# Sara-H-dev/Semantic_Segmentation_Of_StyleGAN2_Artifacts

Measured on AMD Instinct MI355X. Metric: training images/sec at 1024^2 bs=8 per GPU (MS-UNet Swin-T, fwd+DynamicLoss+bwd+AdamW), higher is better.
Workload: dtype bf16; 1 GPU; 1xMI355X 1024x1024 bs=8 Swin-T MS-UNet train step; model=MS-UNet swin_t, global_batch=8, world_size=1, img_size=1024, parallelism=dp1, grad_allreduce=f32, dead_branches=executed (no grad), step_execution=eager, params=42881040

## Files before the change

### include/msunet_hip.h

```cpp
#ifndef MSUNET_HIP_H
#define MSUNET_HIP_H

#ifdef __cplusplus
extern "C" {
#endif

int msu_layernorm_fwd(int dtype, int mode, const void* x, const void* b, const float* bscale,
                      long rows_per_sample, void* s_out, const float* gamma, const float* beta,
                      void* y, float* mean, float* rstd, long rows, int C, int H, int W, int Cin,
                      float eps, void* stream);
int msu_layernorm_bwd(int dtype, int mode, const void* dy, const void* x, const void* dres,
                      const float* gamma, const float* mean, const float* rstd, void* dx,
                      void* db, const float* bscale, long rows_per_sample, float* part,
                      int nparts, float* dgamma, float* dbeta, long rows, int C, int H, int W,
                      int Cin, int accumulate, void* stream);
int msu_layernorm_bwd3(int dtype, int mode, const void* dy, const void* x, const void* dres,
                       const void* dres2, const void* dres3, const float* gamma, const float* mean,
                       const float* rstd, void* dx, void* db, const float* bscale, long rows_per_sample,
                       float* part, int nparts, float* dgamma, float* dbeta, long rows, int C, int H, int W,
                       int Cin, int accumulate, void* stream);
int msu_ln_part_blocks(long rows, int C);
int msu_colsum_batch(int nseg, const float* const* part, const long* stride, const int* nparts, const int* n,
                     float* const* out, int accumulate, void* stream);
int msu_tail_reduce_mode(int mode);
// ... 77 lines not shown
int msu_tok_gemm_supported(long M, int N, int K);
int msu_tok_gemm_supported_epi(long M, int N, int K, int epi);
int msu_tok_gemm(int dtype, const void* A, const void* A2, int K1, const void* W, const float* bias, void* Y,
                 void* Y2, const void* H, long M, int N, int K, int epi, void* stream);
int msu_tok_gemm_plan(long M, int N, int K, long* out6);
int msu_tok_gemm_plan_epi(long M, int N, int K, int epi, int concat, long* out6);
int msu_nt_gemm_supported(long M, int N, int K);
int msu_nt_gemm_plan(long M, int N);
int msu_nt_gemm_plan2(long M, int N, int K, int epi, int wkn, long* out8);
int msu_nt_gemm_mode(int mode);
int msu_nt_gemm(int dtype, const void* A, const void* W, const float* bias, void* Y, void* Y2, const void* H,
                long M, int N, int K, int epi, void* stream);
int msu_nt_gemm_cat(int dtype, const void* A, const void* A2, int K1, const void* W, const float* bias, void* Y,
                    long M, int N, int K, void* stream);
int msu_nt_gemm_kn(int dtype, const void* A, const void* Wk, const float* bias, void* Y, void* Y2, const void* H,
                   long M, int N, int K, int epi, void* stream);

int msu_mlp_fused_supported(int C, int Hd);
int msu_add_ln_mlp_fwd(int dtype, const void* a, const void* br, const float* bscale, long rows_per_sample,
                       const float* gamma, const float* beta, float eps, const void* w1, const float* b1,
                       const void* w2, const float* b2, void* s_out, void* y, long M, int C, int Hd, void* stream);
int msu_mlp_fused_fwd(int dtype, const void* x, const void* w1, const float* b1, const void* w2, const float* b2,
                      void* y, void* h, long M, int C, int Hd, void* stream);
int msu_gelu_fwd(int dtype, const void* x, void* y, long n, void* stream);
int msu_gelu_bwd(int dtype, const void* x, const void* dy, void* dx, long n, void* stream);
int msu_transpose16_multi(const void* src, void* dst, const long long* table, int nent, int ntiles,
                          void* stream);
int msu_residual(int dtype, const void* a, const void* b, const float* scale, void* out, long n, long per_sample,
                 void* stream);
int msu_patchify(int dtype, const float* img, void* out, int B, int Cin, int H, int W, int p,
                 void* stream);

int msu_dynloss_nblk(long N);
int msu_dynloss_fwd(int dtype, const void* logits, const float* target, int B, long N,
                    float alpha, float beta, float mix, float* part, int nblk, float* loss,
                    float* coef, void* stream);
int msu_dynloss_bwd(int dtype, const void* logits, const float* target, const float* coef,
                    const float* loss, const float* gout, int B, long N, float alpha, float beta,
                    float mix, float* dlogits, void* stream);
int msu_dynloss_fwd2(int dtype, const void* logits, const float* target, int B, long N,
                     float alpha, float beta, float mix, float* part, int nblk, float* loss, float* flag,
                     float* coef, void* stream);
int msu_dynloss_bwd2(int dtype, const void* logits, const float* target, const float* coef,
                     const float* flag, const float* gout, int B, long N, float alpha, float beta,
                     float mix, float* dlogits, void* stream);
int msu_dynloss_fwd3(int dtype, const void* logits, const float* target, int B, long N,
// ... 53 lines not shown
```

### semantic_segmentation_of_stylegan2_artifacts_amd/_lib.py

```python
import ctypes
import os

from . import switches

_HERE = os.path.dirname(os.path.abspath(__file__))
LIB_PATH = switches.get("MSU_LIB_OVERRIDE") or os.path.join(_HERE, "libmsunet_hip.so")

P = ctypes.c_void_p
I = ctypes.c_int
L = ctypes.c_long
F = ctypes.c_float
D = ctypes.c_double
U64 = ctypes.c_ulonglong

SIGNATURES = {
    "msu_ln_part_blocks": (I, [L, I]),
    "msu_layernorm_fwd": (I, [I, I, P, P, P, L, P, P, P, P, P, P, L, I, I, I, I, F, P]),
    "msu_layernorm_bwd": (I, [I, I, P, P, P, P, P, P, P, P, P, L, P, I, P, P, L, I, I, I, I, I, P]),
    "msu_layernorm_bwd3": (I, [I, I, P, P, P, P, P, P, P, P, P, P, P, L, P, I, P, P, L, I, I, I, I, I, P]),
    "msu_reduce_rows": (I, [P, I, I, L, P, I, P]),
    "msu_tail_reduce_mode": (I, [I]),
    "msu_conv_mode": (I, [I]),
    "msu_conv3x3_route": (I, [I, I, I]),
    "msu_head_fwd": (I, [I, P, P, P, P, P, P, P, L, I, F, P]),
    "msu_head_bwd": (I, [I, P, P, P, P, P, P, P, P, P, I, P, P, P, L, I, P]),
    "msu_head_bwd2": (I, [I, P, P, P, P, P, P, P, P, P, I, P, P, P, L, I, I, P]),
    "msu_win_count": (L, [I, I, I]),
    "msu_win_attn_fwd_workspace": (L, [I, I, I]),
    "msu_win_attn_keep_words": (L, [I, I, I, I, I]),
    "msu_win_attn_fwd": (I, [I, P, P, P, P, P, I, I, I, I, I, I, F, U64, P, P, P]),
    "msu_win_attn_bwd_workspace": (L, [I, I, I, I, I, I]),
    "msu_win_attn_bwd": (I, [I, P, P, P, P, P, P, P, P, I, I, I, I, I, I, F, U64, P, P, P]),
    "msu_win_attn_bwd2": (I, [I, P, P, P, P, P, P, P, P, I, I, I, I, I, I, F, U64, P, P, P, P]),
    "msu_win_attn_bwd_tail": (I, [I, P, P, P, I, I, I, I, I, P]),
    "msu_win_attn_bwd_tail2": (I, [I, P, P, P, I, I, I, I, I, I, P]),
    "msu_win_attn_qkv_supported": (I, [I, I]),
    "msu_win_attn_qkv_fwd": (I, [I, P, P, P, P, P, P, P, P, I, I, I, I, I, I, F, U64, P, P]),
    "msu_win_attn_qkv_fwd2": (I, [I, P, P, P, P, P, P, P, P, P, P, P, I, I, I, I, I, I, F, U64, P, P]),
    "msu_mlp_fused_supported": (I, [I, I]),
    "msu_mlp_fused_fwd": (I, [I, P, P, P, P, P, P, P, L, I, I, P]),
    "msu_add_ln_mlp_fwd": (I, [I, P, P, P, L, P, P, F, P, P, P, P, P, P, L, I, I, P]),
    "msu_gelu_fwd": (I, [I, P, P, L, P]),
    "msu_gelu_bwd": (I, [I, P, P, P, L, P]),
    "msu_residual": (I, [I, P, P, P, P, L, L, P]),
    "msu_patchify": (I, [I, P, P, I, I, I, I, I, P]),
    "msu_dynloss_nblk": (I, [L]),
    "msu_dynloss_fwd": (I, [I, P, P, I, L, F, F, F, P, I, P, P, P]),
    "msu_dynloss_bwd": (I, [I, P, P, P, P, P, I, L, F, F, F, P, P]),
    "msu_dynloss_fwd2": (I, [I, P, P, I, L, F, F, F, P, I, P, P, P, P]),
    "msu_dynloss_fwd3": (I, [I, P, P, I, L, F, F, F, P, I, P, P, P, P, P]),
    "msu_dynloss_bwd2": (I, [I, P, P, P, P, P, I, L, F, F, F, P, P]),
    "msu_adamw": (I, [P, P, P, P, L, F, F, F, F, F, I, P, P, P]),
    "msu_nonfinite": (I, [P, L, P, P]),
    "msu_nonfinite2": (I, [P, L, P, L, P, P]),
    "msu_grad_sumsq_nblk": (I, [L]),
    "msu_grad_sumsq2": (I, [P, L, P, L, P, I, P, P]),
    "msu_grad_clip_scale": (I, [P, I, P, D, P, P, P]),
    "msu_adamw_dev": (I, [P, P, P, P, L, P, D, D, D, D, P, P, P]),
    "msu_adamw_dev2": (I, [P, P, P, P, L, P, D, D, D, D, P, P, P, I, I, P]),
    "msu_adamw_dev3": (I, [P, P, P, P, P, L, P, D, D, D, D, D, P, P, P, I, I, P]),
    "msu_swap_cast": (I, [P, P, P, I, L, P]),
    "msu_step_advance": (I, [P, P, P]),
    "msu_loss_scale_step": (I, [P, P, P, P, P, P, D, D, I, P]),
# ... 76 lines not shown
```

### semantic_segmentation_of_stylegan2_artifacts_amd/csrc/common.h

```cpp
#pragma once
#include <hip/hip_runtime.h>
#include <hip/hip_bf16.h>
#include <stdint.h>

#include <mutex>

#define MSU_DEV __device__ __forceinline__

typedef __bf16 bf16x8 __attribute__((ext_vector_type(8)));
typedef float f32x4 __attribute__((ext_vector_type(4)));
typedef float f32x16 __attribute__((ext_vector_type(16)));
typedef uint32_t u32x4 __attribute__((ext_vector_type(4)));
typedef uint32_t u32x2 __attribute__((ext_vector_type(2)));
typedef float f32x2 __attribute__((ext_vector_type(2)));
typedef uint16_t bf16_t;
typedef _Float16 f16_t;
typedef _Float16 f16x8 __attribute__((ext_vector_type(8)));

enum MsuDtype { MSU_F32 = 0, MSU_BF16 = 1, MSU_F16 = 2 };

MSU_DEV float to_f32(float v) { return v; }
MSU_DEV float to_f32(bf16_t v) { return __uint_as_float(((uint32_t)v) << 16); }
template <typename T> MSU_DEV T from_f32(float v);
template <> MSU_DEV float from_f32<float>(float v) { return v; }
// ... 112 lines not shown
  const float cdf = 0.5f * (1.0f + erf_fast(x * 0.70710678118654752f, e));
  return fmaf(x * 0.39894228040143268f, e, cdf);
}

MSU_DEV f32x2 pk_fma(f32x2 a, f32x2 b, f32x2 c) { return __builtin_elementwise_fma(a, b, c); }
MSU_DEV f32x2 splat2(float v) { return f32x2{v, v}; }
MSU_DEV f32x2 erf_fast2(f32x2 x, f32x2& e_neg_x2) {
  const f32x2 ax = {fabsf(x.x), fabsf(x.y)};
  const f32x2 d = pk_fma(splat2(0.3275911f), ax, splat2(1.0f));
  const f32x2 t = {__builtin_amdgcn_rcpf(d.x), __builtin_amdgcn_rcpf(d.y)};
  f32x2 p = pk_fma(splat2(1.061405429f), t, splat2(-1.453152027f));
  p = pk_fma(p, t, splat2(1.421413741f));
  p = pk_fma(p, t, splat2(-0.284496736f));
  p = pk_fma(p, t, splat2(0.254829592f)) * t;
  const f32x2 q = -ax * ax;
  e_neg_x2 = f32x2{__expf(q.x), __expf(q.y)};
  const f32x2 r = pk_fma(-p, e_neg_x2, splat2(1.0f));
  return f32x2{copysignf(r.x, x.x), copysignf(r.y, x.y)};
}
MSU_DEV f32x2 gelu_fast2(f32x2 x) {
  f32x2 e;
  return splat2(0.5f) * x * (splat2(1.0f) + erf_fast2(x * splat2(0.70710678118654752f), e));
}

MSU_DEV float hash_uniform(uint64_t seed, uint64_t idx) {
  uint64_t z = seed + 0x9E3779B97F4A7C15ull * (idx + 1);
  z = (z ^ (z >> 30)) * 0xBF58476D1CE4E5B9ull;
  z = (z ^ (z >> 27)) * 0x94D049BB133111EBull;
  z ^= z >> 31;
  return (float)(uint32_t)(z >> 40) * (1.0f / 16777216.0f);
}

MSU_DEV uint64_t launch_seed(uint64_t seed, const unsigned long long* seed_dev) {
  if (seed_dev == nullptr) return seed;
  uint64_t z = seed ^ ((uint64_t)seed_dev[0] * 0x9E3779B97F4A7C15ull);
  z = (z ^ (z >> 31)) * 0xBF58476D1CE4E5B9ull;
  return z ^ (z >> 29);
}

MSU_DEV uint32_t fmix32_hash(uint32_t seed, uint32_t idx) {
  uint32_t x = idx * 0x9E3779B9u + seed;
  x ^= x >> 16; x *= 0x85EBCA6Bu;
  x ^= x >> 13; x *= 0xC2B2AE35u;
  return x ^ (x >> 16);
}
MSU_DEV uint32_t drop_thresh16(float p) { return (uint32_t)ceilf(p * 65536.0f); }
// ... 127 lines not shown
```

### semantic_segmentation_of_stylegan2_artifacts_amd/csrc/mlp_s1.hip

```cpp
#include "common.h"
#include "mfma_frag.h"

namespace {

#ifndef MSU_EXP
#define MSU_EXP 0
#endif

constexpr int SW = 8;
constexpr int STT = 32 * SW;
constexpr int PW = 4, PTT = 32 * PW;
constexpr int UH = 32;
constexpr int FD = (MSU_EXP & 2) ? 1 : 3;
template <bool H_OUT>
constexpr bool s1_h_stores = H_OUT && !(MSU_EXP & 16);

template <int C>
struct S1W {
  static_assert(C == 128 || C == 192 || C == 256, "widths with a register plan and a conflict-free slot image");
  static constexpr int SC = C, SH = 4 * C;
  static constexpr int NU = SH / UH;
  static constexpr int K1 = C / 16;
  static constexpr int NCT = C / 32;
  static constexpr int CPR = C / 8;
  static constexpr int NS = C == 192 ? 6 : C == 256 ? 4 : 8;
  static constexpr int W1S = UH * C;
  static constexpr int W2S = C * UH;
  static constexpr int SLOT = W1S + W2S;
  static constexpr int DMA_W1 = W1S * 2 / 1024;
  static constexpr int DMA_PER_UNIT = SLOT * 2 / 1024;
  static constexpr int DMA_PER_WAVE = DMA_PER_UNIT / SW;
  static_assert(DMA_PER_WAVE * SW == DMA_PER_UNIT, "whole DMA instructions per wave");
  static_assert(NS >= 4 && (NS - 3) * DMA_PER_WAVE + 2 * (NS - 2) <= 63, "steady-state vmcnt fits the counter");
};

template <int C>
struct S1Lds {
  bf16_t ring[S1W<C>::NS * S1W<C>::SLOT];
  float b1[S1W<C>::SH];
  float b2[C];
};
template <int C>
struct S1PLds : S1Lds<C> {
  uint32_t hand[PW][2][2][64 * 4];
};
static_assert(sizeof(S1Lds<128>) <= 160 * 1024 && sizeof(S1Lds<192>) <= 160 * 1024 && sizeof(S1PLds<256>) <= 160 * 1024,
              "LDS");

struct S1Args {
  const bf16_t* x;
  const bf16_t* w1;
  const float* b1;
  const bf16_t* w2;
  const float* b2;
  bf16_t* y;
  bf16_t* hout;
  long M;
};

#define S1_MAP __host__ __device__ __forceinline__ constexpr
S1_MAP int s1_pi(int rho) { return (rho & ~12) | ((rho & 4) << 1) | ((rho & 8) >> 1); }
S1_MAP int w2_swz(int row) { return (row >> 2) & 3; }
template <int C>
S1_MAP int w1_swz(int rho) { return C == 192 ? (rho >> 1) & 7 : rho & 15; }

template <int C>
S1_MAP uint32_t w1_row_off(int rho) { return (uint32_t)(rho * C * 2); }
S1_MAP uint32_t w1_col_off(int c, int sw) { return 16u * (uint32_t)(c ^ sw); }
template <int C>
S1_MAP uint32_t w2_row_off(int row) { return (uint32_t)(S1W<C>::W1S * 2 + row * UH * 2); }
S1_MAP uint32_t w2_col_off(int c, int sw) { return 16u * (uint32_t)(c ^ sw); }
template <int C>
S1_MAP int w1_dma_col(int p) { return (p % S1W<C>::CPR) ^ w1_swz<C>(p / S1W<C>::CPR); }
S1_MAP int w2_dma_col(int p) { return (p & 3) ^ w2_swz(p >> 2); }

constexpr int b128_group_lane(int g, int i) {
  const int l = (g & 1) == 0 ? (i < 4 ? i : i < 8 ? i + 8 : i + 12) : (i < 8 ? i + 4 : i < 12 ? i + 8 : i + 16);
  return l + 32 * (g >> 1);
}
template <int C>
// ... 65 lines not shown
template <int C>
MSU_DEV void s1_dma_unit(const S1Args& A, bf16_t* ring, int wave, int lane, int q, int slot) {
  using W = S1W<C>;
  bf16_t* base = ring + slot * W::SLOT;
  const int ln = opaque(lane);
#pragma unroll
  for (int r = 0; r < W::DMA_PER_WAVE; ++r) {
    const int i = wave + SW * r;
    if (i < W::DMA_W1) {
      const int p = 64 * i + ln, rho = p / W::CPR;
      glds16(A.w1 + (long)(UH * q + s1_pi(rho)) * W::SC + 8 * w1_dma_col<C>(p), base + 512 * i);
    } else {
      const int i2 = i - W::DMA_W1;
      const int p = 64 * i2 + ln, row = p >> 2;
      glds16(A.w2 + (long)row * W::SH + UH * q + 8 * w2_dma_col(p), base + W::W1S + 512 * i2);
    }
  }
}

template <int C>
struct S1Ring {
  using W = S1W<C>;
  static constexpr int NS = W::NS, NU = W::NU, DPW = W::DMA_PER_WAVE;
  static constexpr int steady(bool h_stores) { return (NS - 3) * DPW + (h_stores ? 2 * (NS - 2) : 0); }

  const S1Args& A;
  bf16_t* const ring;
  const int wave, lane;
  const long nunits;
  int issued = 0;
  int mark_x = 0;
  int mark[NS - 2];
  int qn = (NS - 2) % NU, sn = NS - 2;

  MSU_DEV S1Ring(const S1Args& a, bf16_t* r, int w, int l, long n) : A(a), ring(r), wave(w), lane(l), nunits(n) {}

  MSU_DEV void prologue() {
#pragma unroll
    for (int s = 0; s < NS - 2; ++s) {
      if (s < nunits) {
        s1_dma_unit<C>(A, ring, wave, lane, s % NU, s);
        issued += DPW;
      }
      mark[s] = issued;
    }
  }
  template <int STEADY>
  MSU_DEV void wait_chunk() {
    const int younger = issued - mark[0];
    if (younger >= STEADY) wait_vmcnt<STEADY>();
    else wait_vmcnt_le(younger);
  }
  MSU_DEV void refill(long j) {
#pragma unroll
    for (int s = 0; s < NS - 3; ++s) mark[s] = mark[s + 1];
    if (j + NS - 2 < nunits) {
      s1_dma_unit<C>(A, ring, wave, lane, qn, sn);
      issued += DPW;
    }
    mark[NS - 3] = issued;
    qn = qn + 1 == NU ? 0 : qn + 1;
    sn = sn + 1 == NS ? 0 : sn + 1;
  }
  MSU_DEV void count_x() {
    issued += W::K1;
    mark_x = issued;
  }
  MSU_DEV void wait_x() { wait_vmcnt_le(issued - mark_x); }
  MSU_DEV void count_stores(int n) { issued += n; }
};

template <int C>
MSU_DEV void s1_stage_biases(const S1Args& A, S1Lds<C>& L, int tid) {
  for (int s = tid; s < S1W<C>::SH; s += 64 * SW) L.b1[s] = A.b1[s];
  for (int s = tid; s < C; s += 64 * SW) L.b2[s] = A.b2[s];
  __syncthreads();
}

template <typename T, int C>
struct S1Wave {
  using W = S1W<C>;
  static constexpr int SC = W::SC, SH = W::SH, NU = W::NU, K1 = W::K1, NCT = W::NCT, SLOT = W::SLOT;
  const S1Args& A;
  S1Ring<C>& ring;
  const int tl, hh;
  const uint32_t ring0;
  const uint32_t a1_lane;
  const int w1sw;
  const uint32_t a2_lane;
  const int w2sw;
  const uint32_t b1_lane, b2_lane;

  MSU_DEV S1Wave(const S1Args& a, S1Lds<C>& L, S1Ring<C>& r, int lane)
      : A(a), ring(r), tl(lane & 31), hh(lane >> 5), ring0(lds_u32(L.ring)), a1_lane(w1_row_off<C>(tl)),
        w1sw(w1_swz<C>(tl)), a2_lane(w2_row_off<C>(tl)), w2sw(w2_swz(tl)),
        b1_lane(lds_u32(L.b1) + 4u * (uint32_t)(8 * hh)), b2_lane(lds_u32(L.b2) + 4u * (uint32_t)(4 * hh)) {}

  MSU_DEV void load_x(long row0, u32x4 (&xc)[K1]) {
    const long row = row0 + tl;
    const bool ok = row < A.M;
    const bf16_t* p = A.x + (ok ? row : 0) * SC + 8 * hh;
#pragma unroll
    for (int ks = 0; ks < K1; ++ks) {
      const u32x4 v = *reinterpret_cast<const u32x4*>(p + 16 * ks);
      xc[ks] = ok ? v : u32x4{0u, 0u, 0u, 0u};
    }
    ring.count_x();
  }

  MSU_DEV void fc1(int slot, const u32x4 (&xc)[K1], f32x16& h) {
    const uint32_t a1 = ring0 + (uint32_t)(slot * SLOT * 2) + a1_lane;
    h = f32x16{0};
    bf16x8 wf[FD + 1];
    auto addr1 = [&](int ks) { return a1 + w1_col_off(2 * ks + hh, w1sw); };
    unroll_for<FD>([&](auto KS) { wf[decltype(KS)::value] = ds_b128_untracked<0>(addr1(decltype(KS)::value)); });
    unroll_for<K1>([&](auto KS) {
      constexpr int ks = decltype(KS)::value;
      if constexpr (ks + FD < K1) wf[(ks + FD) % (FD + 1)] = ds_b128_untracked<0>(addr1(ks + FD));
      lds_wait_tie<(ks + FD < K1 ? FD : K1 - 1 - ks)>(wf[ks % (FD + 1)]);
      if constexpr (MSU_EXP & 64) {
        const bf16x8 wv = wf[ks % (FD + 1)];
        const u32x4 xv = xc[ks];
        asm volatile("" ::"v"(wv), "v"(xv));
      } else h = Fmt16<T>::mma32(wf[ks % (FD + 1)], __builtin_bit_cast(bf16x8, xc[ks]), h);
    });
  }
  MSU_DEV void fc1_step(int q, int slot, bool more, long next0, u32x4 (&xc)[K1], f32x16& h) {
    if (q == 0) ring.wait_x();
    fc1(slot, xc, h);
    if (q == NU - 1 && more) load_x(next0, xc);
  }

  template <bool H_OUT>
  MSU_DEV void epi(int q, long row0, const f32x16& h, u32x4 (&g)[2]) {
    u32x4 bq[4];
    unroll_for<4>([&](auto BI) {
      constexpr int bi = decltype(BI)::value;
      bq[bi] = __builtin_bit_cast(u32x4, ds_b128_untracked<(bi >> 1) * 64 + (bi & 1) * 16>(
                                             b1_lane + 4u * (uint32_t)(UH * q)));
    });
    lds_wait_tie<0>(bq[0], bq[1], bq[2], bq[3]);
    const long hrow = row0 + tl;
    const bool hok = hrow < A.M;
#pragma unroll
    for (int s = 0; s < 2; ++s) {
      float uu[8];
#pragma unroll
      for (int e = 0; e < 4; ++e) {
        uu[e] = round16<T>(h[8 * s + e] + __uint_as_float(bq[2 * s][e]));
        uu[4 + e] = round16<T>(h[8 * s + 4 + e] + __uint_as_float(bq[2 * s + 1][e]));
      }
      if constexpr (H_OUT) {
        const u32x4 hv = {pack2<T>(uu[0], uu[1]), pack2<T>(uu[2], uu[3]), pack2<T>(uu[4], uu[5]),
                          pack2<T>(uu[6], uu[7])};
        if constexpr (MSU_EXP & 16) {
          const u32x4 hv2 = hv;
          asm volatile("" ::"v"(hv2));
        }
        else if (hok) *reinterpret_cast<u32x4*>(A.hout + hrow * SH + UH * q + 16 * s + 8 * hh) = hv;
      }
      uint32_t gp[4];
#pragma unroll
      for (int e = 0; e < 4; ++e) {
        const f32x2 gv = (MSU_EXP & 8) ? f32x2{uu[2 * e], uu[2 * e + 1]}
                                       : gelu_fast2(f32x2{uu[2 * e], uu[2 * e + 1]});
        gp[e] = pack2<T>(gv.x, gv.y);
      }
      g[s] = u32x4{gp[0], gp[1], gp[2], gp[3]};
    }
    if (s1_h_stores<H_OUT> && row0 + 32 <= A.M) ring.count_stores(2);
  }

  template <bool G_PENDING>
  MSU_DEV void fc2(int slot, u32x4 (&g)[2], f32x16 (&yacc)[NCT]) {
    const uint32_t a2 = ring0 + (uint32_t)(slot * SLOT * 2) + a2_lane;
    auto addr2 = [&](int ct, int s) { return a2 + (uint32_t)(ct * 32 * UH * 2) + w2_col_off(2 * s + hh, w2sw); };
    bf16x8 af[FD + 1];
    unroll_for<FD>([&](auto I) {
      constexpr int i = decltype(I)::value;
      af[i] = ds_b128_untracked<0>(addr2(i % NCT, i / NCT));
    });
    unroll_for<2 * NCT>([&](auto I) {
      constexpr int i = decltype(I)::value, s = i / NCT, ct = i % NCT;
      if constexpr (i + FD < 2 * NCT) af[(i + FD) % (FD + 1)] = ds_b128_untracked<0>(addr2((i + FD) % NCT, (i + FD) / NCT));
      constexpr int behind = i + FD < 2 * NCT ? FD : 2 * NCT - 1 - i;
      if constexpr (G_PENDING && i == 0) lds_wait_tie<behind>(af[0], g[0], g[1]);
      else lds_wait_tie<behind>(af[i % (FD + 1)]);
      if constexpr (MSU_EXP & 32) {
        const bf16x8 av = af[i % (FD + 1)];
        const u32x4 gv = g[s];
        asm volatile("" ::"v"(av), "v"(gv));
      } else yacc[ct] = Fmt16<T>::mma32(af[i % (FD + 1)], __builtin_bit_cast(bf16x8, g[s]), yacc[ct]);
    });
  }

  MSU_DEV void y_out(long row0, f32x16 (&yacc)[NCT]) {
    const long row = row0 + tl;
    const bool ok = row < A.M;
    bf16_t* yr = A.y + (ok ? row : 0) * SC;
#pragma unroll
    for (int ct = 0; ct < NCT; ++ct) {
      uint32_t w[8];
#pragma unroll
      for (int r4 = 0; r4 < 4; ++r4) {
        u32x4 bq;
        asm volatile("ds_read_b128 %0, %1" : "=v"(bq) : "v"(b2_lane + 4u * (uint32_t)(ct * 32 + 8 * r4)));
        lds_wait_tie<0>(bq);
        w[2 * r4] = pack2<T>(yacc[ct][4 * r4] + __uint_as_float(bq[0]), yacc[ct][4 * r4 + 1] + __uint_as_float(bq[1]));
        w[2 * r4 + 1] = pack2<T>(yacc[ct][4 * r4 + 2] + __uint_as_float(bq[2]),
                                 yacc[ct][4 * r4 + 3] + __uint_as_float(bq[3]));
      }
#pragma unroll
      for (int p = 0; p < 2; ++p) {
        const auto s0 = __builtin_amdgcn_permlane32_swap(w[4 * p], w[4 * p + 2], false, false);
        const auto s1 = __builtin_amdgcn_permlane32_swap(w[4 * p + 1], w[4 * p + 3], false, false);
        const u32x4 v = {s0[0], s1[0], s0[1], s1[1]};
        if (ok) *reinterpret_cast<u32x4*>(yr + ct * 32 + 16 * p + 8 * hh) = v;
      }
      yacc[ct] = f32x16{0};
    }
    if (row0 + 32 <= A.M) ring.count_stores(2 * NCT);
  }
};

template <typename T, bool H_OUT, int C>
__global__ void __launch_bounds__(64 * SW) mlp_s1_kernel(S1Args A) {
  using W = S1W<C>;
  using R = S1Ring<C>;
  constexpr int NU = W::NU, NS = W::NS;
  extern __shared__ __attribute__((aligned(16))) unsigned char smem_raw[];
  S1Lds<C>& L = *reinterpret_cast<S1Lds<C>*>(smem_raw);
  const int tid = threadIdx.x, lane = tid & 63;
  const int wave = __builtin_amdgcn_readfirstlane(tid >> 6);
  const long ntiles = (A.M + STT - 1) / STT;
  const int G = gridDim.x;
  const long first = blockIdx.x;
  if (first >= ntiles) return;
  const long mine = (ntiles - 1 - first) / G + 1;
  const long nunits = mine * NU;
  s1_stage_biases<C>(A, L, tid);

  R ring(A, L.ring, wave, lane, nunits);
  S1Wave<T, C> w(A, L, ring, lane);
  auto row0 = [&](long t) { return t * STT + 32 * wave; };
  u32x4 xc[W::K1];
  f32x16 h, yacc[W::NCT];
#pragma unroll
  for (int ct = 0; ct < W::NCT; ++ct) yacc[ct] = f32x16{0};
  w.load_x(row0(first), xc);
  ring.prologue();

  int q = 0, slot = 0;
  long tile = first;
  for (long j = 0; j < nunits; ++j) {
    ring.template wait_chunk<R::steady(s1_h_stores<H_OUT>)>();
    s1_barrier();
    ring.refill(j);
    w.fc1_step(q, slot, tile + G < ntiles, row0(tile + G), xc, h);
    u32x4 g[2];
    w.template epi<H_OUT>(q, row0(tile), h, g);
    w.template fc2<false>(slot, g, yacc);
    if (q == NU - 1) {
      w.y_out(row0(tile), yacc);
      tile += G;
    }
    q = q + 1 == NU ? 0 : q + 1;
    slot = slot + 1 == NS ? 0 : slot + 1;
  }
  wait_vmcnt<0>();
}

template <typename T, bool H_OUT, int C>
__global__ void __launch_bounds__(64 * SW) mlp_s1_kernel_pc(S1Args A) {
  using W = S1W<C>;
  using R = S1Ring<C>;
  constexpr int NU = W::NU, NS = W::NS, K1 = W::K1, NCT = W::NCT, DPW = W::DMA_PER_WAVE;
  static_assert(SW == 2 * PW, "a producer and a consumer per SIMD");
  static_assert(K1 + (NS - 2) * DPW + 2 * (NS - 1) <= 63 && 2 * NCT + (NS - 2) * DPW <= 63, "vmcnt fits the counter");
  extern __shared__ __attribute__((aligned(16))) unsigned char smem_raw[];
  S1PLds<C>& L = *reinterpret_cast<S1PLds<C>*>(smem_raw);
  const int tid = threadIdx.x, lane = tid & 63;
  const int wave = __builtin_amdgcn_readfirstlane(tid >> 6);
  const int pair = wave & (PW - 1);
  const bool producer = wave < PW;
  const long ntiles = (A.M + PTT - 1) / PTT;
  const int G = gridDim.x;
  const long first = blockIdx.x;
  if (first >= ntiles) return;
  const long mine = (ntiles - 1 - first) / G + 1;
  const long nunits = mine * NU;
  s1_stage_biases<C>(A, L, tid);

  R ring(A, L.ring, wave, lane, nunits);
  S1Wave<T, C> w(A, L, ring, lane);
  auto row0 = [&](long t) { return t * PTT + 32 * pair; };
  const uint32_t hand_lane = lds_u32(&L.hand[pair][0][0][0]) + 16u * (uint32_t)lane;

  if (producer) {
    u32x4 xc[K1];
    f32x16 h;
    w.load_x(row0(first), xc);
    ring.prologue();
    int q = 0, slot = 0;
    long tile = first;
    for (long j = 0; j <= nunits; ++j) {
      const bool cur = j < nunits;
      if (cur) ring.template wait_chunk<R::steady(s1_h_stores<H_OUT>)>();
      s1_barrier();
      ring.refill(j);
      if (cur) {
        w.fc1_step(q, slot, tile + G < ntiles, row0(tile + G), xc, h);
        u32x4 g[2];
        w.template epi<H_OUT>(q, row0(tile), h, g);
        asm volatile("ds_write_b128 %0, %1\n\tds_write_b128 %0, %2 offset:1024\n\ts_waitcnt lgkmcnt(0)"
                     :: "v"(hand_lane + 2048u * (uint32_t)(j & 1)), "v"(g[0]), "v"(g[1]) : "memory");
        if (q == NU - 1) tile += G;
        q = q + 1 == NU ? 0 : q + 1;
        slot = slot + 1 == NS ? 0 : slot + 1;
      }
    }
  } else {
    ring.prologue();
    f32x16 yacc[NCT];
#pragma unroll
    for (int ct = 0; ct < NCT; ++ct) yacc[ct] = f32x16{0};
    int qp = 0, slotp = 0;
    long tilep = first;
    for (long j = 0; j <= nunits; ++j) {
      if (j < nunits) ring.template wait_chunk<R::steady(false)>();
      s1_barrier();
      ring.refill(j);
      if (j > 0) {
        const uint32_t hb = hand_lane + 2048u * (uint32_t)((j - 1) & 1);
        u32x4 g[2];
        g[0] = __builtin_bit_cast(u32x4, ds_b128_untracked<0>(hb));
        g[1] = __builtin_bit_cast(u32x4, ds_b128_untracked<1024>(hb));
// ... 6 lines not shown
        slotp = slotp + 1 == NS ? 0 : slotp + 1;
      }
    }
  }
  wait_vmcnt<0>();
}

template <typename T, bool H_OUT, int C>
int launch_s1(const S1Args& a, hipStream_t st) {
  constexpr bool PC = C == 256;
  constexpr int TT = PC ? PTT : STT;
  constexpr size_t LDS = PC ? sizeof(S1PLds<C>) : sizeof(S1Lds<C>);
  void (*kern)(S1Args);
  if constexpr (PC) kern = mlp_s1_kernel_pc<T, H_OUT, C>;
  else kern = mlp_s1_kernel<T, H_OUT, C>;
  static bool attr_set = false;
  if (!attr_set) {
    if (hipFuncSetAttribute((const void*)kern, hipFuncAttributeMaxDynamicSharedMemorySize, (int)LDS) != hipSuccess)
      return -4;
    attr_set = true;
  }
  const long ntiles = (a.M + TT - 1) / TT;
  long grid = msu_num_cus();
  if (grid > ntiles) grid = ntiles;
  hipLaunchKernelGGL(kern, dim3((unsigned)grid), dim3(64 * SW), LDS, st, a);
  return MSU_CHECK_LAUNCH();
}

}

int msu_mlp_s1_width(int C) { return C == 128 || C == 192 || C == 256; }

int msu_mlp_s1_launch(int dtype, const void* x, const void* w1, const float* b1, const void* w2, const float* b2,
                      void* y, void* h, long M, int C, void* stream) {
  S1Args a{};
  a.x = (const bf16_t*)x;
  a.w1 = (const bf16_t*)w1;
  a.b1 = b1;
  a.w2 = (const bf16_t*)w2;
  a.b2 = b2;
  a.y = (bf16_t*)y;
  a.hout = (bf16_t*)h;
  a.M = M;
  hipStream_t st = (hipStream_t)stream;
#define MSU_S1_WIDTH(CC)                                                \
  if (C == CC) {                                                        \
    if (h != nullptr) {                                                 \
      MSU_DISPATCH16(dtype, T, return (launch_s1<T, true, CC>(a, st))); \
    } else {                                                            \
      MSU_DISPATCH16(dtype, T, return (launch_s1<T, false, CC>(a, st)));\
    }                                                                   \
    return -3;                                                          \
  }
  MSU_S1_WIDTH(128)
  MSU_S1_WIDTH(192)
  MSU_S1_WIDTH(256)
#undef MSU_S1_WIDTH
  return -2;
}
```

### semantic_segmentation_of_stylegan2_artifacts_amd/ops.py

```python
import contextlib
import ctypes
import functools

import torch

from . import _lib, switches

_DT = {torch.float32: 0, torch.bfloat16: 1, torch.float16: 2}
_LOW = (torch.bfloat16, torch.float16)


def _dt(t):
    try:
        return _DT[t.dtype]
    except KeyError:
        raise TypeError(f"unsupported activation dtype {t.dtype} (float32 / bfloat16 / float16)") from None


def _need_cuda(*ts):
    for t in ts:
        if t is not None and not t.is_cuda:
            raise RuntimeError("msunet HIP ops need tensors on a HIP device (no CPU fallback)")


# ... 1068 lines not shown
    Hd, C = fc1_weight.shape
    M = x.numel() // C
    if fc2_weight.shape != (C, Hd):
        return False
    return (gemm_route(M, Hd, C, TOK_GELU_DUAL) != "lib" and
            gemm_route(M, Hd, C, TOK_GELU_GRAD) != "lib")


_MLP_INFER = switches.on("MSU_MLP_INFER")
_MLP_TRAIN = switches.on("MSU_MLP_TRAIN")
mlp_infer_calls = 0
mlp_train_calls = 0


MLP_KERNEL_SHAPES = ((96, 384), (192, 768), (128, 512), (256, 1024))
_MLP_S1 = switches.on("MSU_MLP_S1")
MLP_FUSED_SHAPES = MLP_KERNEL_SHAPES if _MLP_S1 else MLP_KERNEL_SHAPES[:1]


def _mlp_fused_ok(C, Hd):
    return (int(C), int(Hd)) in MLP_FUSED_SHAPES


def _mlp_impl(x, w1, b1, w2, b2, keep):
    global mlp_infer_calls, mlp_train_calls
    _need_cuda(x)
    W1 = _shadow(w1, x.dtype)
    W2 = _shadow(w2, x.dtype)
    Hd, C = W1.shape
    fused = _mlp_fused_route(x, w1, keep)
    if fused:
        x = x.contiguous()
        B1, B2 = _f32(b1), _f32(b2)
        if all(t.data_ptr() % 16 == 0 for t in (x, W1, W2, B1, B2)) and W1.is_contiguous() and W2.is_contiguous():
            y = torch.empty(*x.shape[:-1], C, device=x.device, dtype=x.dtype)
            h = torch.empty(*x.shape[:-1], Hd, device=x.device, dtype=x.dtype) if keep else None
            if keep:
                mlp_train_calls += 1
            else:
                mlp_infer_calls += 1
            _lib.call("msu_mlp_fused_fwd", _dt(x), _p(x), _p(W1), _p(B1), _p(W2), _p(B2), _p(y), _p(h),
                      x.numel() // C, C, Hd, _s(x))
            return y, (h if keep else x.new_empty(0)), x.new_empty(0)
    h, g = _gemm(x, W1, _f32(b1), TOK_GELU_DUAL, gelu_only=not keep)
    y = _gemm(g, W2, _f32(b2))
    if not keep:
# ... 20 lines not shown
    ctx.mark_non_differentiable(h, g)
    ctx.set_materialize_grads(False)


def _mlp_backward(ctx, dy, _dh, _dg):
    x, h, g = ctx.saved_tensors
    if dy is None:
        return None, None, None, None, None, None
    if h.numel() == 0:
        raise RuntimeError("mlp: backward through a forward that did not keep its activations (keep=False)")
    w1, b1, w2, b2 = ctx.params
    W1 = _shadow(w1, x.dtype)
    W2 = _shadow(w2, x.dtype)
    dy = _as(dy, x.dtype)
    Hd, C = W1.shape
    M = x.numel() // C
    dy = dy.contiguous()
    if g.numel() == 0:
        dh = _linbwd(dy, h, w2, b2, M, C, Hd, h=h, gelu_x=True)
    else:
        dh = _linbwd(dy, g, w2, b2, M, C, Hd, h=h)
    if dh is None:
        dw2, db2 = _wgrad(dy, g if g.numel() else None, w2, b2, M, C, Hd, x_gelu_of=h)
        dh = _gemm_dx(dy, W2, TOK_GELU_GRAD, h=h, param=w2)
    else:
        dw2 = db2 = None
    dx = _linbwd(dh, x, w1, b1, M, Hd, C) if ctx.needs_input_grad[0] else None
    if dx is None:
        dw1, db1 = _wgrad(dh, x, w1, b1, M, Hd, C)
        dx = _gemm_dx(dh, W1, param=w1) if ctx.needs_input_grad[0] else None
    else:
        dw1 = db1 = None
    return dx, dw1, db1, dw2, db2, None


_mlp = _define("mlp", "(Tensor x, Tensor w1, Tensor b1, Tensor w2, Tensor b2, bool keep) -> (Tensor, Tensor, Tensor)",
               _mlp_impl, _mlp_fake, _mlp_setup, _mlp_backward)


_MLP_LN = switches.on("MSU_MLP_LN")
add_ln_mlp_calls = 0


def add_layer_norm_mlp(a, branch, scale, ln_weight, ln_bias, eps, fc1_weight, fc1_bias, fc2_weight, fc2_bias):
    global add_ln_mlp_calls
    dt = act_dtype()
# ... 636 lines not shown
```

### semantic_segmentation_of_stylegan2_artifacts_amd/switches.py

```python
import os
import warnings

SWITCHES = {
    "MSU_LIB_OVERRIDE": ("", "path of another libmsunet_hip.so (tools/build_exp.sh ablation builds)",
                         "DESIGN 4c"),
    "MSU_WGRAD_SIDE": ("1", "0: every weight gradient on the main stream (determinism bisection)",
                       "DESIGN 4b, 7 (side stream +1.6 %)"),
    "MSU_ATTN_QKV": ("1", "0: the unfused stage-0 qkv Linear + window attention + proj (C = 96 and C = 128)",
                     "DESIGN 4d (r04c: +0.8 % on Swin-T), 7 round 10 (r10a: +0.6 % on Swin-B)"),
    "MSU_GEMM_ROUTE": ("", "force a GEMM route: lib (hipBLASLt) / tok / nt",
                       "DESIGN 7 (r03c: hand-written +2.7 % over hipBLASLt)"),
    "MSU_NT_PP": ("0", "1: the ping-pong NT GEMM (gemm_pp.h) where it tiles exactly, else the persistent one",
                  "DESIGN 7 (r05g: 0.72-0.98x of the persistent kernel; no-store ablation 1.07-1.66x)"),
    "MSU_LINBWD": ("1", "0: stage-0 Linear backward as input-gradient GEMM + side-stream weight gradient",
                   "DESIGN 7 (r03af: one-pass +1.4 %)"),
    "MSU_CONV_SIDE": ("1", "0: the refine-conv weight gradients on the main stream",
                      "DESIGN 7 (r04s: side +0.2 %)"),
    "MSU_TAIL": ("1", "0: LayerNorm parameter-gradient partials summed by a colsum launch, not in the kernel",
                 "DESIGN 7 (r05i: +0.5 %, host -4 ms/step)"),
    "MSU_ATTN_AUX": ("1", "0: each attention backward rebuilds its relative-bias image instead of reusing the "
                     "forward's workspace", "DESIGN 7 (r05az)"),
    "MSU_MLP_INFER": ("1", "0: no-grad stage-0 MLPs on the token-GEMM pair instead of the fused kernel",
                      "DESIGN 7 (r05am: +1.3 %)"),
    "MSU_MLP_LN": ("1", "0: no-grad stage-0 blocks run norm2's residual-add LayerNorm as its own kernel before the "
                   "fused MLP", "DESIGN 7 (r05at)"),
    "MSU_MLP_TRAIN": ("1", "0: training stage-0 MLPs on the token-GEMM pair (H and GELU(H) stored) instead of "
                      "the fused kernel storing H only", "DESIGN 7 (r05ao)"),
    "MSU_LN_DEFER": ("1", "0: each LayerNorm backward sums its parameter-gradient partials itself (in-kernel "
                     "tail) instead of one batched reduction per width", "DESIGN 7 (r06)"),
    "MSU_CONV_DYN": ("1", "0: the refine-conv kernel's static tile schedule (blockIdx.x + k * gridDim.x) instead "
                     "of the device tile queue", "DESIGN 7 (r06)"),
    "MSU_CONV_WGRAD_BLOCKS": ("256", "persistent workgroups of the refine-conv weight gradient (one per CU by "
                              "default; fewer leave CUs to the main stream)", "DESIGN 7 (r04ac, r06)"),
    "MSU_MLP_S1": ("1", "0: the MLPs of the streamed-weight family (Swin-T/S stage 1, 192 -> 768, and Swin-B "
                   "stages 0 and 1, 128 -> 512 and 256 -> 1024; training and no-grad) on the GEMM pair (H and "
                   "GELU(H) stored) instead of the fused kernel streaming its weights through an LDS ring",
                   "DESIGN 7 (r06e, r07a, r08a)"),
    "MSU_RES_HANDOFF": ("1", "0: a stage's first Swin block sums its input's two gradients (norm1 LayerNorm, norm2 "
                        "residual) with an ATen add instead of inside the LayerNorm backward", "DESIGN 7 (r06)"),
    "MSU_GRAPH": ("auto", "HIP-graph replay of the step: 1 / 0 / auto (replay when launch-bound)",
                  "DESIGN 4b (512^2: 401 vs 249-307 img/s)"),
    "MSU_GRAPH_SIDE": ("0", "1: fork the side stream into the captured graph (nondeterministic on ROCm 7.2)",
                       "DESIGN 4b (r03h)"),
}

VALUES = {name: os.environ.get(name, d[0]) for name, d in SWITCHES.items()}


def get(name):
    return VALUES[name]


def on(name):
    return VALUES[name] != "0"


def unknown():
    return sorted(k for k in os.environ if k.startswith("MSU_") and k not in SWITCHES)


# ... 9 lines not shown
```

Before: 183.1 images/s.

## Fuse stage-1 MLP backward into one streamed-weight kernel computing dH and dX

Adds a backward mode to the streamed-weight MLP kernel. From dY it computes dH = (dY·W2ᵀ)·GELU'(H), stores dH for the weight gradient, and computes dX = dH·W1ᵀ in the same pass, reading H through a per-wave LDS buffer. This replaces the token GEMM with a GELU-gradient epilogue plus an NT GEMM that re-read dH from memory. It is enabled by default for the 192->768 and 128->512 shapes when the forward used the fused kernel. The cost is a more complex vmcnt budget and a kernel path that only covers these shapes.

Result: no change. 181.9 images/s (-0.6%).

```diff
diff --git a/include/msunet_hip.h b/include/msunet_hip.h
--- a/include/msunet_hip.h
+++ b/include/msunet_hip.h
@@ -123,6 +123,11 @@
                        const void* w2, const float* b2, void* s_out, void* y, long M, int C, int Hd, void* stream);
 int msu_mlp_fused_fwd(int dtype, const void* x, const void* w1, const float* b1, const void* w2, const float* b2,
                       void* y, void* h, long M, int C, int Hd, void* stream);
+int msu_mlp_s1_bwd_supported(int C, int Hd);
+int msu_mlp_s1_bwd(int dtype, const void* dy, const void* h, const void* w2t, const void* w1t, void* dh, void* dx,
+                   long M, int C, int Hd, void* stream);
+int msu_mlp_s1_bwd_wgs(int dtype, const void* dy, const void* h, const void* w2t, const void* w1t, void* dh,
+                       void* dx, long M, int C, int Hd, int max_wgs, void* stream);
 int msu_gelu_fwd(int dtype, const void* x, void* y, long n, void* stream);
 int msu_gelu_bwd(int dtype, const void* x, const void* dy, void* dx, long n, void* stream);
 int msu_transpose16_multi(const void* src, void* dst, const long long* table, int nent, int ntiles,
diff --git a/semantic_segmentation_of_stylegan2_artifacts_amd/_lib.py b/semantic_segmentation_of_stylegan2_artifacts_amd/_lib.py
--- a/semantic_segmentation_of_stylegan2_artifacts_amd/_lib.py
+++ b/semantic_segmentation_of_stylegan2_artifacts_amd/_lib.py
@@ -39,6 +39,9 @@
     "msu_win_attn_qkv_fwd2": (I, [I, P, P, P, P, P, P, P, P, P, P, P, I, I, I, I, I, I, F, U64, P, P]),
     "msu_mlp_fused_supported": (I, [I, I]),
     "msu_mlp_fused_fwd": (I, [I, P, P, P, P, P, P, P, L, I, I, P]),
+    "msu_mlp_s1_bwd_supported": (I, [I, I]),
+    "msu_mlp_s1_bwd": (I, [I, P, P, P, P, P, P, L, I, I, P]),
+    "msu_mlp_s1_bwd_wgs": (I, [I, P, P, P, P, P, P, L, I, I, I, P]),
     "msu_add_ln_mlp_fwd": (I, [I, P, P, P, L, P, P, F, P, P, P, P, P, P, L, I, I, P]),
     "msu_gelu_fwd": (I, [I, P, P, L, P]),
     "msu_gelu_bwd": (I, [I, P, P, P, L, P]),
diff --git a/semantic_segmentation_of_stylegan2_artifacts_amd/csrc/common.h b/semantic_segmentation_of_stylegan2_artifacts_amd/csrc/common.h
--- a/semantic_segmentation_of_stylegan2_artifacts_amd/csrc/common.h
+++ b/semantic_segmentation_of_stylegan2_artifacts_amd/csrc/common.h
@@ -158,6 +158,11 @@
   f32x2 e;
   return splat2(0.5f) * x * (splat2(1.0f) + erf_fast2(x * splat2(0.70710678118654752f), e));
 }
+MSU_DEV f32x2 gelu_grad_fast2(f32x2 x) {
+  f32x2 e;
+  const f32x2 cdf = splat2(0.5f) * (splat2(1.0f) + erf_fast2(x * splat2(0.70710678118654752f), e));
+  return pk_fma(x * splat2(0.39894228040143268f), e, cdf);
+}
 
 MSU_DEV float hash_uniform(uint64_t seed, uint64_t idx) {
   uint64_t z = seed + 0x9E3779B97F4A7C15ull * (idx + 1);
diff --git a/semantic_segmentation_of_stylegan2_artifacts_amd/csrc/mlp_s1.hip b/semantic_segmentation_of_stylegan2_artifacts_amd/csrc/mlp_s1.hip
--- a/semantic_segmentation_of_stylegan2_artifacts_amd/csrc/mlp_s1.hip
+++ b/semantic_segmentation_of_stylegan2_artifacts_amd/csrc/mlp_s1.hip
@@ -1,3 +1,5 @@
+#include <type_traits>
+
 #include "common.h"
 #include "mfma_frag.h"
 
@@ -31,8 +33,11 @@
   static constexpr int DMA_PER_UNIT = SLOT * 2 / 1024;
   static constexpr int DMA_PER_WAVE = DMA_PER_UNIT / SW;
   static_assert(DMA_PER_WAVE * SW == DMA_PER_UNIT, "whole DMA instructions per wave");
-  static_assert(NS >= 4 && (NS - 3) * DMA_PER_WAVE + 2 * (NS - 2) <= 63, "steady-state vmcnt fits the counter");
+  static_assert(NS >= 4 && (NS - 3) * DMA_PER_WAVE + 2 * (NS - 2) + 2 * (NS - 3) <= 63,
+                "steady-state vmcnt fits the counter");
 };
+
+enum S1Mode { S1_FWD = 0, S1_FWD_H = 1, S1_BWD = 2 };
 
 template <int C>
 struct S1Lds {
@@ -41,10 +46,16 @@
   float b2[C];
 };
 template <int C>
+struct S1BLds {
+  bf16_t ring[S1W<C>::NS * S1W<C>::SLOT];
+  bf16_t hbuf[SW][2 * 512];
+};
+template <int C>
 struct S1PLds : S1Lds<C> {
   uint32_t hand[PW][2][2][64 * 4];
 };
-static_assert(sizeof(S1Lds<128>) <= 160 * 1024 && sizeof(S1Lds<192>) <= 160 * 1024 && sizeof(S1PLds<256>) <= 160 * 1024,
+static_assert(sizeof(S1Lds<128>) <= 160 * 1024 && sizeof(S1Lds<192>) <= 160 * 1024 && sizeof(S1PLds<256>) <= 160 * 1024 &&
+                  sizeof(S1BLds<128>) <= 160 * 1024 && sizeof(S1BLds<192>) <= 160 * 1024,
               "LDS");
 
 struct S1Args {
@@ -56,6 +67,7 @@
   bf16_t* y;
   bf16_t* hout;
   long M;
+  const bf16_t* hin;
 };
 
 #define S1_MAP __host__ __device__ __forceinline__ constexpr
@@ -167,7 +179,9 @@
 struct S1Ring {
   using W = S1W<C>;
   static constexpr int NS = W::NS, NU = W::NU, DPW = W::DMA_PER_WAVE;
-  static constexpr int steady(bool h_stores) { return (NS - 3) * DPW + (h_stores ? 2 * (NS - 2) : 0); }
+  static constexpr int steady(bool h_stores, bool h_loads = false) {
+    return (NS - 3) * DPW + (h_stores ? 2 * (NS - 2) : 0) + (h_loads ? 2 * (NS - 3) : 0);
+  }
 
   const S1Args& A;
   bf16_t* const ring;
@@ -175,6 +189,7 @@
   const long nunits;
   int issued = 0;
   int mark_x = 0;
+  int mark_h = 0;
   int mark[NS - 2];
   int qn = (NS - 2) % NU, sn = NS - 2;
 
@@ -213,6 +228,11 @@
   }
   MSU_DEV void wait_x() { wait_vmcnt_le(issued - mark_x); }
   MSU_DEV void count_stores(int n) { issued += n; }
+  MSU_DEV void count_h() {
+    issued += 2;
+    mark_h = issued;
+  }
+  MSU_DEV void wait_h() { wait_vmcnt_le(issued - mark_h); }
 };
 
 template <int C>
@@ -236,10 +256,11 @@
   const int w2sw;
   const uint32_t b1_lane, b2_lane;
 
-  MSU_DEV S1Wave(const S1Args& a, S1Lds<C>& L, S1Ring<C>& r, int lane)
-      : A(a), ring(r), tl(lane & 31), hh(lane >> 5), ring0(lds_u32(L.ring)), a1_lane(w1_row_off<C>(tl)),
+  MSU_DEV S1Wave(const S1Args& a, const bf16_t* lds_ring, const float* lds_b1, const float* lds_b2, S1Ring<C>& r,
+                 int lane)
+      : A(a), ring(r), tl(lane & 31), hh(lane >> 5), ring0(lds_u32(lds_ring)), a1_lane(w1_row_off<C>(tl)),
         w1sw(w1_swz<C>(tl)), a2_lane(w2_row_off<C>(tl)), w2sw(w2_swz(tl)),
-        b1_lane(lds_u32(L.b1) + 4u * (uint32_t)(8 * hh)), b2_lane(lds_u32(L.b2) + 4u * (uint32_t)(4 * hh)) {}
+        b1_lane(lds_u32(lds_b1) + 4u * (uint32_t)(8 * hh)), b2_lane(lds_u32(lds_b2) + 4u * (uint32_t)(4 * hh)) {}
 
   MSU_DEV void load_x(long row0, u32x4 (&xc)[K1]) {
     const long row = row0 + tl;
@@ -276,8 +297,10 @@
     if (q == NU - 1 && more) load_x(next0, xc);
   }
 
-  template <bool H_OUT>
+  template <int MODE>
   MSU_DEV void epi(int q, long row0, const f32x16& h, u32x4 (&g)[2]) {
+    static_assert(MODE == S1_FWD || MODE == S1_FWD_H, "the backward form: epi_bwd");
+    constexpr bool H_OUT = MODE == S1_FWD_H;
     u32x4 bq[4];
     unroll_for<4>([&](auto BI) {
       constexpr int bi = decltype(BI)::value;
@@ -314,6 +337,36 @@
       g[s] = u32x4{gp[0], gp[1], gp[2], gp[3]};
     }
     if (s1_h_stores<H_OUT> && row0 + 32 <= A.M) ring.count_stores(2);
+  }
+
+  MSU_DEV void load_h(int q, long row0, bf16_t* hbuf) {
+    const long hrow = row0 + tl;
+    const bf16_t* p = A.hin + (hrow < A.M ? hrow : 0) * SH + UH * q + 8 * hh;
+    glds16(p, hbuf);
+    glds16(p + 16, hbuf + 512);
+    ring.count_h();
+  }
+  MSU_DEV void read_h(const bf16_t* hbuf, u32x4 (&hc)[2]) {
+    const uint32_t a = lds_u32(hbuf) + 16u * (uint32_t)(tl + 32 * hh);
+    hc[0] = __builtin_bit_cast(u32x4, ds_b128_untracked<0>(a));
+    hc[1] = __builtin_bit_cast(u32x4, ds_b128_untracked<1024>(a));
+    lds_wait_tie<0>(hc[0], hc[1]);
+  }
+  MSU_DEV void epi_bwd(int q, long row0, const f32x16& h, const u32x4 (&hc)[2], u32x4 (&g)[2]) {
+    const long hrow = row0 + tl;
+    const bool hok = hrow < A.M;
+#pragma unroll
+    for (int s = 0; s < 2; ++s) {
+      uint32_t gp[4];
+#pragma unroll
+      for (int e = 0; e < 4; ++e) {
+        const f32x2 gg = gelu_grad_fast2(f32x2{Fmt16<T>::lo(hc[s][e]), Fmt16<T>::hi(hc[s][e])});
+        gp[e] = pack2<T>(h[8 * s + 2 * e] * gg.x, h[8 * s + 2 * e + 1] * gg.y);
+      }
+      g[s] = u32x4{gp[0], gp[1], gp[2], gp[3]};
+      if (hok) *reinterpret_cast<u32x4*>(A.hout + hrow * SH + UH * q + 16 * s + 8 * hh) = g[s];
+    }
+    if (row0 + 32 <= A.M) ring.count_stores(2);
   }
 
   template <bool G_PENDING>
@@ -339,6 +392,7 @@
     });
   }
 
+  template <bool BIAS = true>
   MSU_DEV void y_out(long row0, f32x16 (&yacc)[NCT]) {
     const long row = row0 + tl;
     const bool ok = row < A.M;
@@ -348,9 +402,11 @@
       uint32_t w[8];
 #pragma unroll
       for (int r4 = 0; r4 < 4; ++r4) {
-        u32x4 bq;
-        asm volatile("ds_read_b128 %0, %1" : "=v"(bq) : "v"(b2_lane + 4u * (uint32_t)(ct * 32 + 8 * r4)));
-        lds_wait_tie<0>(bq);
+        u32x4 bq = {0u, 0u, 0u, 0u};
+        if constexpr (BIAS) {
+          asm volatile("ds_read_b128 %0, %1" : "=v"(bq) : "v"(b2_lane + 4u * (uint32_t)(ct * 32 + 8 * r4)));
+          lds_wait_tie<0>(bq);
+        }
         w[2 * r4] = pack2<T>(yacc[ct][4 * r4] + __uint_as_float(bq[0]), yacc[ct][4 * r4 + 1] + __uint_as_float(bq[1]));
         w[2 * r4 + 1] = pack2<T>(yacc[ct][4 * r4 + 2] + __uint_as_float(bq[2]),
                                  yacc[ct][4 * r4 + 3] + __uint_as_float(bq[3]));
@@ -368,13 +424,15 @@
   }
 };
 
-template <typename T, bool H_OUT, int C>
-__global__ void __launch_bounds__(64 * SW) mlp_s1_kernel(S1Args A) {
+template <typename T, int MODE, int C>
+MSU_DEV void s1_one_role(const S1Args& A) {
   using W = S1W<C>;
   using R = S1Ring<C>;
   constexpr int NU = W::NU, NS = W::NS;
+  constexpr bool BWD = MODE == S1_BWD;
+  using Lds = std::conditional_t<BWD, S1BLds<C>, S1Lds<C>>;
   extern __shared__ __attribute__((aligned(16))) unsigned char smem_raw[];
-  S1Lds<C>& L = *reinterpret_cast<S1Lds<C>*>(smem_raw);
+  Lds& L = *reinterpret_cast<Lds*>(smem_raw);
   const int tid = threadIdx.x, lane = tid & 63;
   const int wave = __builtin_amdgcn_readfirstlane(tid >> 6);
   const long ntiles = (A.M + STT - 1) / STT;
@@ -383,36 +441,60 @@
   if (first >= ntiles) return;
   const long mine = (ntiles - 1 - first) / G + 1;
   const long nunits = mine * NU;
-  s1_stage_biases<C>(A, L, tid);
+  const float *lds_b1 = nullptr, *lds_b2 = nullptr;
+  bf16_t* hbuf = nullptr;
+  if constexpr (BWD) hbuf = L.hbuf[wave];
+  else {
+    s1_stage_biases<C>(A, L, tid);
+    lds_b1 = L.b1;
+    lds_b2 = L.b2;
+  }
 
   R ring(A, L.ring, wave, lane, nunits);
-  S1Wave<T, C> w(A, L, ring, lane);
+  S1Wave<T, C> w(A, L.ring, lds_b1, lds_b2, ring, lane);
   auto row0 = [&](long t) { return t * STT + 32 * wave; };
   u32x4 xc[W::K1];
   f32x16 h, yacc[W::NCT];
 #pragma unroll
   for (int ct = 0; ct < W::NCT; ++ct) yacc[ct] = f32x16{0};
   w.load_x(row0(first), xc);
+  if constexpr (BWD) w.load_h(0, row0(first), hbuf);
   ring.prologue();
 
   int q = 0, slot = 0;
   long tile = first;
   for (long j = 0; j < nunits; ++j) {
-    ring.template wait_chunk<R::steady(s1_h_stores<H_OUT>)>();
+    ring.template wait_chunk<R::steady(BWD || s1_h_stores<MODE == S1_FWD_H>, BWD)>();
     s1_barrier();
+    u32x4 hc[2];
+    if constexpr (BWD) {
+      ring.wait_h();
+      w.read_h(hbuf, hc);
+      if (j + 1 < nunits) w.load_h(q + 1 == NU ? 0 : q + 1, row0(q + 1 == NU ? tile + G : tile), hbuf);
+    }
     ring.refill(j);
     w.fc1_step(q, slot, tile + G < ntiles, row0(tile + G), xc, h);
     u32x4 g[2];
-    w.template epi<H_OUT>(q, row0(tile), h, g);
+    if constexpr (BWD) w.epi_bwd(q, row0(tile), h, hc, g);
+    else w.template epi<MODE>(q, row0(tile), h, g);
     w.template fc2<false>(slot, g, yacc);
     if (q == NU - 1) {
-      w.y_out(row0(tile), yacc);
+      w.template y_out<!BWD>(row0(tile), yacc);
       tile += G;
     }
     q = q + 1 == NU ? 0 : q + 1;
     slot = slot + 1 == NS ? 0 : slot + 1;
   }
   wait_vmcnt<0>();
+}
+
+template <typename T, bool H_OUT, int C>
+__global__ void __launch_bounds__(64 * SW) mlp_s1_kernel(S1Args A) {
+  s1_one_role<T, H_OUT ? S1_FWD_H : S1_FWD, C>(A);
+}
+template <typename T, int C>
+__global__ void __launch_bounds__(64 * SW) mlp_s1_bwd_kernel(S1Args A) {
+  s1_one_role<T, S1_BWD, C>(A);
 }
 
 template <typename T, bool H_OUT, int C>
@@ -437,7 +519,7 @@
   s1_stage_biases<C>(A, L, tid);
 
   R ring(A, L.ring, wave, lane, nunits);
-  S1Wave<T, C> w(A, L, ring, lane);
+  S1Wave<T, C> w(A, L.ring, L.b1, L.b2, ring, lane);
   auto row0 = [&](long t) { return t * PTT + 32 * pair; };
   const uint32_t hand_lane = lds_u32(&L.hand[pair][0][0][0]) + 16u * (uint32_t)lane;
 
@@ -456,7 +538,7 @@
       if (cur) {
         w.fc1_step(q, slot, tile + G < ntiles, row0(tile + G), xc, h);
         u32x4 g[2];
-        w.template epi<H_OUT>(q, row0(tile), h, g);
+        w.template epi<H_OUT ? S1_FWD_H : S1_FWD>(q, row0(tile), h, g);
         asm volatile("ds_write_b128 %0, %1\n\tds_write_b128 %0, %2 offset:1024\n\ts_waitcnt lgkmcnt(0)"
                      :: "v"(hand_lane + 2048u * (uint32_t)(j & 1)), "v"(g[0]), "v"(g[1]) : "memory");
         if (q == NU - 1) tile += G;
@@ -509,6 +591,24 @@
   }
   const long ntiles = (a.M + TT - 1) / TT;
   long grid = msu_num_cus();
+  if (grid > ntiles) grid = ntiles;
+  hipLaunchKernelGGL(kern, dim3((unsigned)grid), dim3(64 * SW), LDS, st, a);
+  return MSU_CHECK_LAUNCH();
+}
+
+template <typename T, int C>
+int launch_s1_bwd(const S1Args& a, int max_wgs, hipStream_t st) {
+  constexpr size_t LDS = sizeof(S1BLds<C>);
+  void (*kern)(S1Args) = mlp_s1_bwd_kernel<T, C>;
+  static bool attr_set = false;
+  if (!attr_set) {
+    if (hipFuncSetAttribute((const void*)kern, hipFuncAttributeMaxDynamicSharedMemorySize, (int)LDS) != hipSuccess)
+      return -4;
+    attr_set = true;
+  }
+  const long ntiles = (a.M + STT - 1) / STT;
+  long grid = msu_num_cus();
+  if (max_wgs > 0 && grid > max_wgs) grid = max_wgs;
   if (grid > ntiles) grid = ntiles;
   hipLaunchKernelGGL(kern, dim3((unsigned)grid), dim3(64 * SW), LDS, st, a);
   return MSU_CHECK_LAUNCH();
@@ -545,3 +645,38 @@
 #undef MSU_S1_WIDTH
   return -2;
 }
+
+extern "C" {
+
+int msu_mlp_s1_bwd_supported(int C, int Hd) { return (C == 128 || C == 192) && Hd == 4 * C ? 1 : 0; }
+
+int msu_mlp_s1_bwd_wgs(int dtype, const void* dy, const void* h, const void* w2t, const void* w1t, void* dh, void* dx,
+                       long M, int C, int Hd, int max_wgs, void* stream) {
+  if (!msu_is16(dtype) || !msu_mlp_s1_bwd_supported(C, Hd) || M < 0) return -2;
+  if (dy == nullptr || h == nullptr || w2t == nullptr || w1t == nullptr || dh == nullptr || dx == nullptr) return -2;
+  if ((((uintptr_t)dy | (uintptr_t)h | (uintptr_t)w2t | (uintptr_t)w1t | (uintptr_t)dh | (uintptr_t)dx) & 15) != 0)
+    return -2;
+  if (M == 0) return 0;
+  S1Args a{};
+  a.x = (const bf16_t*)dy;
+  a.w1 = (const bf16_t*)w2t;
+  a.w2 = (const bf16_t*)w1t;
+  a.y = (bf16_t*)dx;
+  a.hout = (bf16_t*)dh;
+  a.hin = (const bf16_t*)h;
+  a.M = M;
+  hipStream_t st = (hipStream_t)stream;
+  if (C == 128) {
+    MSU_DISPATCH16(dtype, T, return (launch_s1_bwd<T, 128>(a, max_wgs, st)));
+  } else {
+    MSU_DISPATCH16(dtype, T, return (launch_s1_bwd<T, 192>(a, max_wgs, st)));
+  }
+  return -3;
+}
+
+int msu_mlp_s1_bwd(int dtype, const void* dy, const void* h, const void* w2t, const void* w1t, void* dh, void* dx,
+                   long M, int C, int Hd, void* stream) {
+  return msu_mlp_s1_bwd_wgs(dtype, dy, h, w2t, w1t, dh, dx, M, C, Hd, 0, stream);
+}
+
+}
diff --git a/semantic_segmentation_of_stylegan2_artifacts_amd/ops.py b/semantic_segmentation_of_stylegan2_artifacts_amd/ops.py
--- a/semantic_segmentation_of_stylegan2_artifacts_amd/ops.py
+++ b/semantic_segmentation_of_stylegan2_artifacts_amd/ops.py
@@ -1114,6 +1114,28 @@
     return (int(C), int(Hd)) in MLP_FUSED_SHAPES
 
 
+MLP_S1_BWD_SHAPES = ((192, 768), (128, 512))
+_MLP_S1_BWD = switches.on("MSU_MLP_S1_BWD")
+mlp_s1_bwd_calls = 0
+
+
+def _mlp_s1_bwd_ok(C, Hd, fused_fwd, needs_dx, wt2, wt1):
+    return bool(_MLP_S1_BWD and fused_fwd and needs_dx and wt2 is not None and wt1 is not None and
+                (int(C), int(Hd)) in MLP_S1_BWD_SHAPES and (int(C), int(Hd)) in MLP_FUSED_SHAPES[1:])
+
+
+def _mlp_s1_bwd(dy, h, wt2, wt1, M, C, Hd):
+    global mlp_s1_bwd_calls
+    ts = (dy, h, wt2, wt1)
+    if not all(t.is_contiguous() and t.data_ptr() % 16 == 0 for t in ts):
+        return None
+    dh = torch.empty_like(h)
+    dx = torch.empty(*dy.shape[:-1], C, device=dy.device, dtype=dy.dtype)
+    _lib.call("msu_mlp_s1_bwd", _dt(dy), _p(dy), _p(h), _p(wt2), _p(wt1), _p(dh), _p(dx), M, C, Hd, _s(dy))
+    mlp_s1_bwd_calls += 1
+    return dh, dx
+
+
 def _mlp_impl(x, w1, b1, w2, b2, keep):
     global mlp_infer_calls, mlp_train_calls
     _need_cuda(x)
@@ -1180,6 +1202,12 @@
         dh = _linbwd(dy, g, w2, b2, M, C, Hd, h=h)
     if dh is None:
         dw2, db2 = _wgrad(dy, g if g.numel() else None, w2, b2, M, C, Hd, x_gelu_of=h)
+        wt2, wt1 = _shadow_t(w2, x.dtype), _shadow_t(w1, x.dtype)
+        if _mlp_s1_bwd_ok(C, Hd, g.numel() == 0, ctx.needs_input_grad[0], wt2, wt1):
+            both = _mlp_s1_bwd(dy, h, wt2, wt1, M, C, Hd)
+            if both is not None:
+                dw1, db1 = _wgrad(both[0], x, w1, b1, M, Hd, C)
+                return both[1], dw1, db1, dw2, db2, None
         dh = _gemm_dx(dy, W2, TOK_GELU_GRAD, h=h, param=w2)
     else:
         dw2 = db2 = None
diff --git a/semantic_segmentation_of_stylegan2_artifacts_amd/switches.py b/semantic_segmentation_of_stylegan2_artifacts_amd/switches.py
--- a/semantic_segmentation_of_stylegan2_artifacts_amd/switches.py
+++ b/semantic_segmentation_of_stylegan2_artifacts_amd/switches.py
@@ -36,6 +36,9 @@
                    "stages 0 and 1, 128 -> 512 and 256 -> 1024; training and no-grad) on the GEMM pair (H and "
                    "GELU(H) stored) instead of the fused kernel streaming its weights through an LDS ring",
                    "DESIGN 7 (r06e, r07a, r08a)"),
+    "MSU_MLP_S1_BWD": ("1", "0: the backward of the one-role streamed-weight MLPs (192 -> 768, 128 -> 512) as the "
+                       "GEMM pair (token GEMM with the GELU-gradient epilogue, then the NT GEMM re-reading dH) "
+                       "instead of one kernel computing dH and dX from dY", "DESIGN 7 (r20a)"),
     "MSU_RES_HANDOFF": ("1", "0: a stage's first Swin block sums its input's two gradients (norm1 LayerNorm, norm2 "
                         "residual) with an ATen add instead of inside the LayerNorm backward", "DESIGN 7 (r06)"),
     "MSU_GRAPH": ("auto", "HIP-graph replay of the step: 1 / 0 / auto (replay when launch-bound)",
```
